# TLeconte/vdlm2dec

Measured on AMD Instinct MI355X. Metric: IQ MS/s demodulated (8 ch, 2 MS/s cs16) + CRC-pass frame parity vs ref, higher is better.
Workload: dtype f32

## Files before the change

vdlm2dec_amd/csrc/vdl2gpu_scan.h:

```cpp
#ifndef VDL2GPU_SCAN_H
#define VDL2GPU_SCAN_H

#ifndef K2A_THREADS
#define K2A_THREADS 256
#endif
#ifndef K2A_TS
#define K2A_TS 1024
#endif
#ifndef K2A_WPE
#define K2A_WPE 6
#endif
#define K2A_POFF 132
#define K2A_XOFF (K2A_POFF + 16)
#define K2A_XMAX (2 * K2A_TS + K2A_XOFF)
#define K2X_WL 40
#define K2X_NT 256
#define K2X_CV 64
#define VDL2_ITEM_CAP 196608
#define VDL2_ITEM_PRIV 131072
#define VDL2_MAXWG 512
#define VDL2_REG_CAP 4096
#ifndef VDL2_REG_PAD
#define VDL2_REG_PAD 40
#endif
#ifndef VDL2_REG_GAP
#define VDL2_REG_GAP 96
#endif
#define VDL2_SEG_CAP 4096
#define VDL2_VERIFIED 0x7f000000
#define VDL2_SEED_ERR 7.0f

struct K2aDef {
	int n;
	int r;
	int lo, hi;
};

#define K2A_ITEM_WORDS 5
struct K2aItem { float4 w[K2A_ITEM_WORDS]; };

#define K2A_WU1 (K2A_TS + K2A_XOFF + 4)
#define K2A_XS_LEN (K2A_WU1 + K2A_TS + K2A_POFF + 4)
struct alignas(16) K2aShared {
	float2 xs[K2A_XS_LEN];
	float smf[72];
	unsigned it_used, it_limit;
	unsigned short pend[K2A_THREADS / 64][K2A_TS / (K2A_THREADS / 64)];
	unsigned long long prof[K2A_ST_SLOTS];
};
static_assert(K2A_WU1 % 2 == 0 && K2A_XS_LEN >= K2A_XMAX + 8 && (K2A_XMAX / 2 + 4) % 2 == 0, "16-byte reads of xs[] and wu[]");
static_assert(K2A_TS + K2A_POFF / 2 + 2 <= K2A_XS_LEN && K2A_WU1 >= K2A_TS + K2A_XOFF, "phasor areas");
static_assert(K2A_TS <= 1024, "pend[] holds an instant within the tile in ten bits");
#define K2A_XODD (K2A_XMAX / 2 + 4)

#define VDL2_SCREEN_R2 56.25f
#define VDL2_SCREEN_R22 42.25f
#define VDL2_SCREEN_R32 30.25f
#define VDL2_FIT_MARGIN 0.25f
#define VDL2_NB_MARGIN 0.1f
__device__ __forceinline__ float k2_fast_angle(float y, float x)
{
	const float ax = __builtin_fabsf(x), ay = __builtin_fabsf(y);
	const float mn = __builtin_fminf(ax, ay), mx = __builtin_fmaxf(ax, ay);
	const float t = mn * __builtin_amdgcn_rcpf(mx);
	const float s = t * t;
	float p = __fmaf_rn(s, -0.0117212f, 0.05265332f);
	p = __fmaf_rn(s, p, -0.11643287f);
	p = __fmaf_rn(s, p, 0.19354346f);
	p = __fmaf_rn(s, p, -0.33262347f);
	p = __fmaf_rn(s, p, 0.99997726f) * t;
	p = ay > ax ? 1.57079637f - p : p;
	p = x < 0.0f ? 3.14159274f - p : p;
	return __builtin_copysignf(p, y);
}

__device__ __forceinline__ v2f k2_rot(v2f acc, v2f u, float cx, float cy)
{
	acc = __builtin_elementwise_fma((v2f){cx, cx}, u, acc);
	return __builtin_elementwise_fma((v2f){-cy, cy}, u.yx, acc);
}


template <class PR> __device__ __forceinline__ void k2a_emit(PR p, int sc, long long dec_base, long long n, int r, int mode,
						  long long chk_lo, long long chk_hi, int *fail, int skip_r, int skip_par,
						  float p2err, float perr, float err, float pfr, unsigned *cntp, unsigned *ovf, Cand *cl)
{
	if (mode >= SURV_PROBE && perr < VDL2_SEED_ERR && err > perr) {
		const unsigned kk = atomicAdd(p.ctl + CTL_NSEED0(p) + sc, 1u);
		if (kk < VDL2_CAND_CAP)
			p.seeds[(size_t)sc * VDL2_CAND_CAP + kk] = (int)(n - dec_base);
	}
	if (mode == SURV_SEEDS_NEVER_SET)
		return;
	if (!(perr < 4.0f && err > perr))
		return;
	if (mode == SURV_CANDS || mode == SURV_PROBE) {
		if (r == skip_r && (int)(n & 1) == skip_par)
			return;
		if (p.round == 0 && !p.full_scan && p2err < 4.0f && perr > p2err)
			return;
	} else {
		if (n < chk_lo || n >= chk_hi)
			return;
		atomicMin(fail, (int)(n - dec_base));
		const unsigned kc = atomicAdd(cntp, 1u);
		if (kc < VDL2_CAND_CAP) {
			Cand cd;
			cd.nrel = (int)(n - dec_base);
			cd.r = r;
			cd.p2err = p2err;
			cd.perr = perr;
			cd.err = err;
			cd.pfr = pfr;
			cl[kc] = cd;
			p.clhead[(size_t)sc * VDL2_CAND_CAP + kc] = cl_pack(0, CL_INVALID, 0, 0, 0, 0, 0);
		} else
			*ovf = 1u;
		return;
	}
	const unsigned kk = atomicAdd(cntp, 1u);
	if (kk < VDL2_CAND_CAP) {
		Cand cd;
		cd.nrel = (int)(n - dec_base);
		cd.r = r;
		cd.p2err = p2err;
		cd.perr = perr;
		cd.err = err;
		cd.pfr = pfr;
		cl[kk] = cd;
	} else
		*ovf = 1u;
}

__device__ __forceinline__ void k2a_tables(K2aShared &sh)
{
	for (int i = threadIdx.x; i < 72; i += K2A_THREADS)
		sh.smf[i] = (i < 65) ? d_tab(c_mflt, i) : 0.0f;
	if (threadIdx.x == 0) {
		sh.it_used = 0;
		sh.it_limit = 0xffffffffu;
	}
	__syncthreads();
}


__device__ __forceinline__ void k2a_append(K2aShared &sh, const K2Params &p, int sc, bool pass, int n_rel, int r, int lo, int hi, const float2 (&uu)[16], bool odd, int mode, int *fail)
{
	const unsigned long long m = __ballot(pass);
	if (m == 0)
		return;
	const unsigned lane_rank = __builtin_amdgcn_mbcnt_hi((unsigned)(m >> 32), __builtin_amdgcn_mbcnt_lo((unsigned)m, 0u));
	const unsigned cnt = (unsigned)__popcll(m);
	unsigned base = 0, stride = 0;
	if (lane_rank == 0 && pass) {
		const unsigned pch = (unsigned)p.surv_pch;
		const unsigned off = atomicAdd(&sh.it_used, cnt);
		if (off + cnt <= pch) {
			base = blockIdx.x * pch * K2A_ITEM_WORDS + off;
			stride = pch;
		} else {
			atomicMin(&sh.it_limit, off);
			const unsigned priv = (unsigned)p.surv_nwg * pch;
			const unsigned off2 = atomicAdd(p.ctl + CTL_NSURV0(p) + p.surv_slot * p.nstreams * VDL2_CS + sc, cnt);
			stride = p.item_cap - priv;
			const unsigned room = (p.surv_common_cap > 0 && (unsigned)p.surv_common_cap < stride) ? (unsigned)p.surv_common_cap : stride;
			base = (off2 + cnt <= room) ? priv * K2A_ITEM_WORDS + off2 : 0xffffffffu;
			if (base == 0xffffffffu)
				atomicMax(p.ctl + CTL_NSURVLIM0(p) + p.surv_slot * p.nstreams * VDL2_CS + sc, ~off2);
		}
	}
	const int lead = __builtin_ctzll(m);
	base = (unsigned)__builtin_amdgcn_readlane((int)base, lead);
	stride = (unsigned)__builtin_amdgcn_readlane((int)stride, lead);
	if (!pass)
		return;
	if (base != 0xffffffffu) {
		float4 *dst = reinterpret_cast<float4 *>(p.items) + (size_t)sc * p.item_cap * K2A_ITEM_WORDS + base + lane_rank;
		dst[0] = make_float4(__int_as_float(n_rel), __int_as_float(r | (odd ? 0x100 : 0)), __int_as_float(lo), __int_as_float(hi));
#pragma unroll
		for (int w = 0; w < 4; ++w) {
			typedef short s2 __attribute__((ext_vector_type(2)));
			union { s2 v; int i; } c[4];
#pragma unroll
			for (int l = 0; l < 4; ++l)
				c[l].v = __builtin_amdgcn_cvt_pknorm_i16(uu[4 * w + l].x, uu[4 * w + l].y);
			dst[(size_t)(1 + w) * stride] = make_float4(__int_as_float(c[0].i), __int_as_float(c[1].i), __int_as_float(c[2].i), __int_as_float(c[3].i));
		}
	} else if (mode == SURV_VERIFY)
		atomicMin(fail, 0);
	else
// ... 294 lines not shown
		v2f xe[10], xo[10];
#pragma unroll
		for (int i = 0; i < 5; ++i) {
			xe[2 * i] = e[i].xy;
			xe[2 * i + 1] = e[i].zw;
			xo[2 * i] = o[i].xy;
			xo[2 * i + 1] = o[i].zw;
		}
#pragma unroll
		for (int m = 0; m < 9; ++m) {
			acc0 = __builtin_elementwise_fma(xe[m], (v2f){mf[2 * m], mf[2 * m]}, acc0);
			acc1 = __builtin_elementwise_fma(xe[m + 1], (v2f){mf[2 * m], mf[2 * m]}, acc1);
			if (m < 8) {
				acc0 = __builtin_elementwise_fma(xo[m], (v2f){mf[2 * m + 1], mf[2 * m + 1]}, acc0);
				acc1 = __builtin_elementwise_fma(xo[m + 1], (v2f){mf[2 * m + 1], mf[2 * m + 1]}, acc1);
			}
		}
	} else {
		const v4f *pe = reinterpret_cast<const v4f *>(&sh.xs[q0]);
		v4f e[9];
#pragma unroll
		for (int i = 0; i < 9; ++i)
			e[i] = pe[i];
		v2f x[18];
#pragma unroll
		for (int i = 0; i < 9; ++i) {
			x[2 * i] = e[i].xy;
			x[2 * i + 1] = e[i].zw;
		}
#pragma unroll
		for (int j = 0; j < 17; ++j) {
			acc0 = __builtin_elementwise_fma(x[j], (v2f){mf[j], mf[j]}, acc0);
			acc1 = __builtin_elementwise_fma(x[j + 1], (v2f){mf[j], mf[j]}, acc1);
		}
	}
}

__device__ __forceinline__ v2f k2a_unit(v2f a)
{
	const float n2 = __fmaf_rn(a.x, a.x, a.y * a.y);
	v2f w = a * __frsqrt_rn(n2);
	if (!(n2 >= 1e-30f && n2 <= 1e30f)) {
		const float bad = (a.x == 0.0f && a.y == 0.0f) ? 0.0f : __builtin_nanf("");
		w = (v2f){1.0f + bad, bad};
	}
	return w;
}

__device__ __forceinline__ float k2a_lane_from(int byte_addr, float v)
{
	return __int_as_float(__builtin_amdgcn_ds_bpermute(byte_addr, __float_as_int(v)));
}

template <int S> __device__ void k2a_tile(K2aShared &sh, const K2Params &p, int sc, long long dec_base, long long nbase,
					   int cnt, unsigned rmask, int mode, long long chk_lo, long long chk_hi, int *fail,
					   int skip_r = -1, int skip_par = 0)
{
	const int tid = threadIdx.x;
	constexpr int PH = K2A_POFF / S;
	constexpr int LSTR = 8 / S;
	constexpr int E2 = 2 / S, E4 = 4 / S;
	constexpr int KH = LSTR / 2;
	constexpr int PPW = 64 - KH;
	constexpr int PPI = (K2A_THREADS / 64) * PPW;
	constexpr int NIT = ((K2A_TS + PH + 1) / 2 + PPI - 1) / PPI;
	constexpr int NL = (S * (K2A_TS - 1) + 1 + K2A_XOFF + K2A_THREADS - 1) / K2A_THREADS;
	static_assert(K2A_POFF == S * PH, "phase history must be a whole number of instants");
	float2 *const wu = (S != 1) ? sh.xs : sh.xs + K2A_WU1;
	const int nx = S * (cnt - 1) + 1 + K2A_XOFF;
	const bool prof = p.dbg && (mode == SURV_PROBE || (mode == SURV_CANDS && S == 1 && !p.full_scan && !p.full_round)) && tid == 0 && (blockIdx.x & 7) == 0;
	long long tq = prof ? clock64() : 0;
#define K2A_STAMP(slot) do { if (prof) { const long long tn = clock64(); sh.prof[slot] += (unsigned long long)(tn - tq); tq = tn; } } while (0)
	const int pbase = (S == 2) ? (tid & 1) * K2A_XODD + (tid >> 1) : tid;
	constexpr int pstep = K2A_THREADS / S;
	{
		const float2 *x = p.dec + (size_t)sc * p.cap + (nbase - K2A_XOFF - dec_base);
		float2 v[NL];
#pragma unroll
		for (int k = 0; k < NL; ++k)
			if (tid + k * K2A_THREADS < nx)
				v[k] = x[tid + k * K2A_THREADS];
		K2A_STAMP(K2A_ST_TILES_OR_WAIT);
#pragma unroll
		for (int k = 0; k < NL; ++k)
			if (tid + k * K2A_THREADS < nx)
				sh.xs[pbase + k * pstep] = v[k];
	}
	K2A_STAMP(K2A_ST_PARK);
	__syncthreads();
	K2A_STAMP(K2A_ST_STAGE_IN);
	const int npairs = (cnt + PH + 1) / 2;
	const int wv = tid >> 6, ln = tid & 63;
	const int src_lane = (ln - KH) * 4;
#pragma unroll 1
	for (int r = 0; r < 4; ++r) {
		if (!(rmask & (1u << r)))
			continue;
		float mf[17];
#pragma unroll
		for (int j = 0; j < 17; ++j)
			mf[j] = __int_as_float(__builtin_amdgcn_readfirstlane(__float_as_int(sh.smf[r + 4 * j])));
		float4 hold[NIT];
#pragma unroll
		for (int it = 0; it < NIT; ++it) {
			const int pw = it * PPI + wv * PPW;
			if (pw >= npairs) {
				hold[it] = make_float4(0.0f, 0.0f, 0.0f, 0.0f);
				continue;
			}
			int q0 = 2 * (pw + ln - KH);
			q0 = q0 < 0 ? 0 : (q0 > K2A_TS + PH - 2 ? K2A_TS + PH - 2 : q0);
			v2f acc[2];
			k2a_fir2<S>(sh, q0, mf, acc[0], acc[1]);
			const v2f w0 = k2a_unit(acc[0]), w1 = k2a_unit(acc[1]);
			const float p0x = k2a_lane_from(src_lane, w0.x), p0y = k2a_lane_from(src_lane, w0.y);
			const float p1x = k2a_lane_from(src_lane, w1.x), p1y = k2a_lane_from(src_lane, w1.y);
			hold[it] = make_float4(__fmaf_rn(w0.x, p0x, w0.y * p0y), __fmaf_rn(w0.y, p0x, -(w0.x * p0y)),
					       __fmaf_rn(w1.x, p1x, w1.y * p1y), __fmaf_rn(w1.y, p1x, -(w1.x * p1y)));
			__builtin_amdgcn_sched_barrier(0);
		}
		K2A_STAMP(K2A_ST_FIR_UNIT);
		if (S != 1)
			__syncthreads();
		K2A_STAMP(K2A_ST_BARRIER_SAMPLES);
#pragma unroll
		for (int it = 0; it < NIT; ++it) {
			const int q0 = 2 * (it * PPI + wv * PPW + ln - KH);
			if (ln >= KH && q0 >= LSTR && q0 < cnt + PH)
				*reinterpret_cast<float4 *>(&wu[q0]) = hold[it];
		}
		K2A_STAMP(K2A_ST_STEPS);
		__syncthreads();
		unsigned npend = 0;
		for (int i0 = 0; i0 < cnt; i0 += K2A_THREADS) {
			const int i = i0 + tid;
			const int j = (i < cnt ? i : cnt - 1) + E2;
			const float2 *uq = &wu[PH - E4 + j - 15 * LSTR];
			float2 uu[16];
#pragma unroll
			for (int l = 0; l < 16; ++l)
				uu[l] = uq[l * LSTR];
			constexpr int kq[16] = {7, 4, 5, 3, 7, 6, 1, 3, 6, 0, 5, 2, 1, 2, 0, 4};
			v2f s4[4] = {{0.0f, 0.0f}, {0.0f, 0.0f}, {0.0f, 0.0f}, {0.0f, 0.0f}};
#pragma unroll
			for (int l = 0; l < 16; ++l) {
				const v2f u = {uu[l].x, uu[l].y};
				const int g = ((kq[l] & 1) << 1) | ((kq[l] >> 1) & 1);
				if (kq[l] & 4)
					s4[g] -= u;
				else
					s4[g] += u;
			}
			const v2f pa = {s4[0].x - s4[1].y, s4[0].y + s4[1].x};
			const v2f qa = {s4[2].x - s4[3].y, s4[2].y + s4[3].x};
			constexpr float RH = 0.70710678118654752f;
			const v2f acc = {__fmaf_rn(qa.x - qa.y, RH, pa.x), __fmaf_rn(qa.x + qa.y, RH, pa.y)};
			const float r2 = __fmaf_rn(acc.x, acc.x, acc.y * acc.y);
			bool pass = i < cnt && !(r2 <= VDL2_SCREEN_R2);
			if (mode == SURV_CANDS && r == skip_r && (int)((nbase + S * (j - E4)) & 1) == skip_par)
				pass = false;
			const unsigned long long m = __ballot(pass);
			if (m != 0) {
				if (pass)
					sh.pend[wv][npend + __builtin_amdgcn_mbcnt_hi((unsigned)(m >> 32), __builtin_amdgcn_mbcnt_lo((unsigned)m, 0u))] =
						(unsigned short)(i | (!(r2 == r2) ? 0x8000 : 0));
				npend += (unsigned)__popcll(m);
			}
		}
		for (unsigned b = 0; b < npend; b += 64) {
			const bool on = b + (unsigned)ln < npend;
			const int e = on ? (int)sh.pend[wv][b + (unsigned)ln] : 0;
			const int j = (e & 0x3ff) + E2;
			const float2 *uq = &wu[PH - E4 + j - 15 * LSTR];
			float2 uu[16];
#pragma unroll
			for (int l = 0; l < 16; ++l)
				uu[l] = uq[l * LSTR];
			const long long n_abs = nbase + S * (j - E4);
			k2a_append(sh, p, sc, on, (int)(n_abs - dec_base), r, (mode == SURV_VERIFY) ? (int)(chk_lo - dec_base) : 0,
				   (mode == SURV_VERIFY) ? (int)(chk_hi - dec_base) : 0, uu, (e & 0x8000) != 0, mode, fail);
		}
		K2A_STAMP(K2A_ST_SCREEN);
		K2A_STAMP(K2A_ST_SCREEN_END);
		__syncthreads();
		K2A_STAMP(K2A_ST_BARRIER_TILE);
		if (prof)
			sh.prof[K2A_ST_PASSES] += 1ull;
	}
#undef K2A_STAMP
}

__global__ __launch_bounds__(K2A_THREADS) __attribute__((amdgpu_waves_per_eu(K2A_WPE, 8)))
void k2a_probe(K2Params p)
{
	__shared__ K2aShared sh;
	const int c = blockIdx.y, s = (int)blockIdx.z;
	const int sc = s * VDL2_CS + c;
	const long long dec_base = p.dec_base;
	const long long avail_end = dec_base + VDL2_CARRY_FRAMES + p.J;
	if (p.force_serial)
		return;
	if (p.round > 0 && (!p.full_round || p.fail[sc] >= VDL2_VERIFIED))
		return;
	if (threadIdx.x < K2A_ST_SLOTS)
		sh.prof[threadIdx.x] = 0;
	k2a_tables(sh);
	if (p.full_scan || p.full_round) {
		const long long step = (long long)gridDim.x * K2A_TS;
		for (long long n0 = p.scan_lo + (long long)blockIdx.x * K2A_TS; n0 < avail_end; n0 += step) {
			const int nt = (int)((avail_end - n0 < K2A_TS) ? (avail_end - n0) : K2A_TS);
			k2a_tile<1>(sh, p, sc, dec_base, n0, nt, 0xfu, SURV_CANDS, 0, 0, nullptr);
		}
		k2a_tail(sh, sc);
		return;
	}
	const unsigned rmask = 1u << p.probe_r;
	const long long step = 2LL * gridDim.x * K2A_TS;
	for (long long n0 = p.scan_lo + 2LL * blockIdx.x * K2A_TS; n0 < avail_end; n0 += step) {
		const long long left = (avail_end - n0 + 1) / 2;
		const int nt = (int)(left < K2A_TS ? left : K2A_TS);
		k2a_tile<2>(sh, p, sc, dec_base, n0, nt, rmask, SURV_PROBE, 0, 0, nullptr);
	}
	k2a_tail(sh, sc);
	if (p.dbg && threadIdx.x < K2A_ST_SLOTS && sh.prof[threadIdx.x])
		atomicAdd(p.dbg + K2_DBG_PROBE_STAGE0 + threadIdx.x, sh.prof[threadIdx.x]);
}

#define WGS_NBK 2048
#define WGS_MAXB 48
struct WgSortShared {
	unsigned long long tmp[VDL2_CAND_CAP];
	unsigned start[WGS_NBK + 1], cur[WGS_NBK];
	unsigned part[64];
	unsigned maxb;
};

template <int NT> __device__ void wg_sort_u64(unsigned long long *keys, WgSortShared &ws, int n, int tshift, unsigned range)
{
	const int tid = threadIdx.x;
	int bsh = 0;
	while ((range >> bsh) >= WGS_NBK)
		++bsh;
	for (int b = tid; b < WGS_NBK; b += NT)
		ws.cur[b] = 0;
	if (tid == 0)
		ws.maxb = 0;
	__syncthreads();
	for (int i = tid; i < n; i += NT) {
		unsigned b = (unsigned)(keys[i] >> tshift) >> bsh;
		b = b < WGS_NBK ? b : WGS_NBK - 1;
		const unsigned k = atomicAdd(&ws.cur[b], 1u);
		if (k + 1 > WGS_MAXB)
			ws.maxb = 1;
	}
	__syncthreads();
	if (ws.maxb) {
		int npow = 1;
		while (npow < n)
			npow <<= 1;
		for (int i = n + tid; i < npow; i += NT)
			keys[i] = ~0ull;
		__syncthreads();
		for (int k = 2; k <= npow; k <<= 1)
			for (int j = k >> 1; j > 0; j >>= 1) {
				for (int i = tid; i < npow; i += NT) {
					const int l = i ^ j;
					if (l > i) {
						const unsigned long long a0 = keys[i], b0 = keys[l];
						if ((a0 > b0) == ((i & k) == 0)) {
							keys[i] = b0;
							keys[l] = a0;
						}
					}
				}
// ... 106 lines not shown
				continue;
			int j = i;
			while (j + 1 < ncand && key[j + 1] - key[j] <= VDL2_REG_GAP)
				++j;
			int lo = key[i] - VDL2_REG_PAD, hi = key[j] + VDL2_REG_PAD + 1;
			lo = lo < lo_lim ? lo_lim : lo;
			hi = hi > hi_lim ? hi_lim : hi;
			if (hi <= lo)
				continue;
			const int nchunk = (hi - lo + K2A_TS - 1) / K2A_TS;
			const int base = atomicAdd(&s_nreg, nchunk);
			for (int k = 0; k < nchunk; ++k)
				if (base + k < VDL2_REG_CAP) {
					const int q = lo + k * K2A_TS;
					regs[base + k] = make_int2(q, (hi - q < K2A_TS) ? hi - q : K2A_TS);
				}
		}
		__syncthreads();
#ifdef VDL2GPU_TESTHOOKS
		if (K2_REG_LIM(p) < VDL2_REG_CAP && s_nreg > K2_REG_LIM(p)) {
			const int n = s_nreg < VDL2_REG_CAP ? s_nreg : VDL2_REG_CAP, lim = K2_REG_LIM(p);
			for (int i = tid; i < n; i += K2R_NT)
				key64[i] = ((unsigned long long)(unsigned)regs[i].x << 32) | (unsigned)regs[i].y;
			__syncthreads();
			for (int i = tid; i < n; i += K2R_NT) {
				const int x = (int)(key64[i] >> 32);
				int rank = 0;
				for (int j = 0; j < n; ++j)
					rank += ((int)(key64[j] >> 32) < x) ? 1 : 0;
				const int k = (int)(((long long)rank * lim + n - 1) / n);
				if (k < lim && (int)((long long)k * n / lim) == rank)
					regs[k] = make_int2(x, (int)(key64[i] & 0xffffffffu));
			}
			__syncthreads();
		}
#endif
		if (tid == 0) {
			const int n = s_nreg;
			p.ctl[CTL_NREG0(p) + sc] = (unsigned)(n > K2_REG_LIM(p) ? K2_REG_LIM(p) : n);
			if (n > K2_REG_LIM(p))
				K2_COUNT(p, K2_DBG_ESC_REG);
			p.ctl[CTL_NSEED0(p) + sc] = 0;
		}
	}
}

#ifndef K2A_WPE_REGION
#define K2A_WPE_REGION 5
#endif
__global__ __launch_bounds__(K2A_THREADS) __attribute__((amdgpu_waves_per_eu(K2A_WPE_REGION, 8)))
void k2a_region(K2Params p)
{
	__shared__ K2aShared sh;
	const int c = blockIdx.y, s = (int)blockIdx.z;
	const int sc = s * VDL2_CS + c;
	if (p.force_serial || p.full_scan)
		return;
#ifdef VDL2GPU_TESTHOOKS
	if (p.test_noregion && p.round == 0)
		return;
#endif
	const unsigned nreg = p.ctl[CTL_NREG0(p) + sc];
	if (blockIdx.x >= nreg)
		return;
	const long long dec_base = p.dec_base;
	const int2 *regs = p.regs + (size_t)sc * VDL2_REG_CAP;
	const int skip_r = p.probe_r, skip_par = p.probe_par;
	if (threadIdx.x < K2A_ST_SLOTS)
		sh.prof[threadIdx.x] = 0;
	k2a_tables(sh);
	const bool prof = p.dbg && threadIdx.x == 0 && (blockIdx.x & 7) == 0;
	const long long t0 = prof ? clock64() : 0;
	for (unsigned k = blockIdx.x; k < nreg; k += gridDim.x) {
		const int2 rg = regs[k];
		k2a_tile<1>(sh, p, sc, dec_base, dec_base + rg.x, rg.y, 0xfu, SURV_CANDS, 0, 0, nullptr, skip_r, skip_par);
		if (prof)
			sh.prof[K2A_ST_INSTANTS] += (unsigned long long)rg.y;
	}
	const long long t1 = prof ? clock64() : 0;
	if (prof)
		sh.prof[K2A_ST_TILES_OR_WAIT] += (unsigned long long)(t1 - t0);
	k2a_tail(sh, sc);
	if (p.dbg && threadIdx.x < K2A_ST_SLOTS && sh.prof[threadIdx.x])
		atomicAdd(p.dbg + K2_DBG_REGION_STAGE0 + threadIdx.x, sh.prof[threadIdx.x]);
}

#ifndef K2A_VRUN
#define K2A_VRUN 4
#endif
#ifndef K2A_VGRID_RESIDENT
#define K2A_VGRID_RESIDENT 1
#endif
#define K2A_VITEMS 64

__device__ __forceinline__ int k2a_vseg(const Seg *segs, int k, int nseg, int p_lo, int t_end, int &lo, int &hi, int &r)
{
	lo = hi = r = 0;
	if (k >= nseg)
		return 0;
	const Seg g = segs[k];
	lo = g.lo > p_lo ? g.lo : p_lo;
	lo += (lo ^ g.lo) & 1;
	hi = g.hi < t_end ? g.hi : t_end;
	r = g.r & 3;
	if (g.hi <= g.lo || hi <= lo) {
		hi = lo;
		return 0;
	}
	return ((hi - lo + 1) / 2 + K2A_TS - 1) / K2A_TS;
}

__device__ __forceinline__ int k2a_vscan(int v, int *s_w, int &total)
{
	int incl = v;
	incl += __builtin_amdgcn_update_dpp(0, incl, 0x111, 0xf, 0xf, false);
	incl += __builtin_amdgcn_update_dpp(0, incl, 0x112, 0xf, 0xf, false);
	incl += __builtin_amdgcn_update_dpp(0, incl, 0x114, 0xf, 0xf, false);
	incl += __builtin_amdgcn_update_dpp(0, incl, 0x118, 0xf, 0xf, false);
	incl += __builtin_amdgcn_update_dpp(0, incl, 0x142, 0xa, 0xf, false);
	incl += __builtin_amdgcn_update_dpp(0, incl, 0x143, 0xc, 0xf, false);
	__syncthreads();
	if ((threadIdx.x & 63) == 63)
		s_w[threadIdx.x >> 6] = incl;
	__syncthreads();
	int base = 0, tot = 0;
#pragma unroll
	for (int w = 0; w < K2A_THREADS / 64; ++w) {
		const int t = s_w[w];
// ... 31 lines not shown
}

__global__ __launch_bounds__(K2A_THREADS) __attribute__((amdgpu_waves_per_eu(K2A_WPE, 8)))
void k2a_verify(K2Params p)
{
	__shared__ K2aShared sh;
	__shared__ int s_w[K2A_THREADS / 64];
	__shared__ int4 s_item[K2A_VITEMS];
	const int tid = threadIdx.x;
	const int c = blockIdx.y, s = (int)blockIdx.z;
	const int sc = s * VDL2_CS + c;
	if (p.force_serial || p.full_scan || p.full_round)
		return;
	if (p.round > 0 && !p.redo[sc])
		return;
	const long long dec_base = p.dec_base;
	const int t_end = (int)(VDL2_CARRY_FRAMES + p.J);
	int nseg = (int)p.ctl[CTL_NSEG0(p) + sc];
	if (tid == 0 && blockIdx.x == 0 && (nseg < 0 || nseg > K2_SEG_LIM(p)))
		K2_COUNT(p, K2_DBG_ESC_SEG);
	nseg = nseg < 0 || nseg > K2_SEG_LIM(p) ? K2_SEG_LIM(p) : nseg;
	const Seg *segs = p.segs + (size_t)sc * VDL2_SEG_CAP;
	if (nseg == 0)
		return;
	const int p_lo = (int)(p.cs[sc].pos - dec_base);
	int lo0, hi0, r0;
	const int n0 = k2a_vseg(segs, tid, nseg, p_lo, t_end, lo0, hi0, r0);
	int T;
	{
		int mine = n0;
		for (int k = K2A_THREADS + tid; k < nseg; k += K2A_THREADS) {
			int lo, hi, r;
			mine += k2a_vseg(segs, k, nseg, p_lo, t_end, lo, hi, r);
		}
		k2a_vscan(mine, s_w, T);
	}
	const int G = (int)gridDim.x;
	const int q = (T + G - 1) / G;
	int ch = (int)blockIdx.x;
	int a = ch * q;
	if (a >= T)
		return;
	int c_end = a + q < T ? a + q : T;
	k2a_tables(sh);
	int b = a + K2A_VITEMS < c_end ? a + K2A_VITEMS : c_end;
	k2a_vitems<true>(segs, nseg, p_lo, t_end, a, b, lo0, hi0, r0, n0, s_w, s_item);
	for (;;) {
		const int ni = b - a;
		if (p.dbg && tid < ni)
			atomicAdd(p.dbg + K2_DBG_VERIFY_INSTANTS, (unsigned long long)((s_item[tid].y - s_item[tid].x + 1) / 2));
		for (int i = 0; i < ni; ++i) {
			const int4 it = s_item[i];
			k2a_tile<2>(sh, p, sc, dec_base, dec_base + it.x, (it.y - it.x + 1) / 2, 1u << it.z, SURV_VERIFY, dec_base + it.x, dec_base + it.y,
				    p.fail + sc);
		}
		a = b;
		if (a >= c_end) {
			ch += G;
			a = ch * q;
			if (a >= T)
				break;
			c_end = a + q < T ? a + q : T;
		}
		b = a + K2A_VITEMS < c_end ? a + K2A_VITEMS : c_end;
		__syncthreads();
		k2a_vitems<false>(segs, nseg, p_lo, t_end, a, b, 0, 0, 0, 0, s_w, s_item);
	}
	k2a_tail(sh, sc);
}

#endif
```

vdlm2dec_amd/csrc/vdl2gpu_types.h:

```cpp
#ifndef VDL2GPU_TYPES_H
#define VDL2GPU_TYPES_H


#include <hip/hip_runtime.h>
#include <stdint.h>
#include "vdl2_math.h"
#include "../../include/vdl2gpu.h"

#define VDL2_CS 8
#ifndef VDL2_NSET
#define VDL2_NSET 3
#endif
#define VDL2_NRING VDL2_NSET
#define VDL2_NSLAB (VDL2_NSET + 1)
static_assert(VDL2_NSET >= 3 && VDL2_NSET <= 4, "three bits of a record handle name its slab");
#define VDL2_HIST 160
#define VDL2_NPH 68
#define VDL2_STEADY 68
#define VDL2_MAXSYM 5456
#define VDL2_SERIAL_BELOW 4096
#define VDL2_CARRY_FRAMES 49152
#define VDL2_LONGEST_BURST 43592
#define VDL2_LEV_GUARD 512
#define VDL2_LEV_NEVAL 256
// ... 205 lines not shown
	vdl2gpu_soft_t *soft;
	RingCount *outc;
	OutCounters::Totals *outc_total;
	unsigned *fmask;
	int full_round;
	int mini_round;
	int sel_reserved;
	unsigned rec_cap;
	int force_serial;
	int prim_drop;
	int full_scan;
	int test_noregion;
	int2 *regs;
	Seg *segs;
	int *fail;
	int *redo;
	int round;
	ChanState *cs_out;
	int *skey;
	unsigned short *sidx;
	unsigned short *prim;
	uint8_t *onchain;
	K2Slog *slog;
	int2 *win;
	int *seeds;
	struct K2aItem *items;
	unsigned item_cap;
	unsigned item_priv;
	int surv_pch, surv_nwg;
	int surv_common_cap;
	int surv_slot;
	int surv_mode;
	int surv_skip;
	int drain_slot;
	int drain_mode, drain_skip;
	int drain_pch, drain_nwg;
	unsigned long long *dbg;
	HeadTap *headtap;
	unsigned *headtap_n;
	unsigned headtap_cap;
	vdl2gpu_carrier_t *carrier;
#ifdef VDL2GPU_TESTHOOKS
	int lim_reg, lim_seg, lim_vis, lim_win, lim_merge, lim_slog;
#endif
};
enum K2Dbg {
	K2_DBG_K2B_RING_TICKS = 0, K2_DBG_K2B_REST_TICKS, K2_DBG_K2B_SAMPLED, K2_DBG_K2B_TRIG, K2_DBG_K2B_EVAL, K2_DBG_K2B_MAX_TICKS,
	K2_DBG_K2B_STEADY, K2_DBG_K2B_REJ, K2_DBG_K2B_ORD_TICKS0 = 8, K2_DBG_K2B_ORD_COUNT0 = 12,
	K2_DBG_K2C_LOAD_TICKS = 16, K2_DBG_K2C_TABLES_TICKS, K2_DBG_K2C_WALK_TICKS, K2_DBG_K2C_PUBLISH_TICKS, K2_DBG_K2C_CALLS,
	K2_DBG_REPAIRED = 24, K2_DBG_K2C_REPLAYS, K2_DBG_K2C_NONSTEADY, K2_DBG_K2C_CANDS, K2_DBG_K2C_VISITED, K2_DBG_K2C_SERIAL_SAMPLES,
	K2_DBG_VERIFY_INSTANTS = 30, K2_DBG_PROBE_STAGE0 = 32, K2_DBG_REGION_STAGE0 = 48,
	K2_DBG_ESC_REG = 64, K2_DBG_ESC_SEG, K2_DBG_ESC_VIS, K2_DBG_ESC_WIN, K2_DBG_ESC_MERGE, K2_DBG_ESC_SLOG, K2_DBG_ESC_STAGE,
	K2_DBG_INV_B_CLUSTER, K2_DBG_INV_B_DECODE, K2_DBG_INV_B_RECORD, K2_DBG_INV_A, K2_DBG_ESC_MERGE_SORT,
	K2_DBG_ESC_PATCH_ABANDON, K2_DBG_CHK_B_CLUSTER, K2_DBG_CHK_B_DECODE, K2_DBG_CHK_B_RECORD, K2_DBG_CHK_A
};
enum K2aStage {
	K2A_ST_STAGE_IN = 0, K2A_ST_FIR_UNIT, K2A_ST_BARRIER_SAMPLES, K2A_ST_STEPS, K2A_ST_SCREEN, K2A_ST_UNUSED5, K2A_ST_UNUSED6, K2A_ST_UNUSED7,
	K2A_ST_SCREEN_END, K2A_ST_BARRIER_TILE, K2A_ST_UNUSED10, K2A_ST_PASSES , K2A_ST_TILES_OR_WAIT, K2A_ST_PARK, K2A_ST_UNUSED14,
	K2A_ST_INSTANTS , K2A_ST_SLOTS
};
static_assert(K2A_ST_SLOTS == 16 && K2_DBG_REGION_STAGE0 == K2_DBG_PROBE_STAGE0 + K2A_ST_SLOTS && K2_DBG_ESC_REG == K2_DBG_REGION_STAGE0 + K2A_ST_SLOTS,
	      "the two scans' stage slots lie between the resolver's counters and the test build's");
#ifdef VDL2GPU_TESTHOOKS
#define K2_REG_LIM(p) ((p).lim_reg)
#define K2_SEG_LIM(p) ((p).lim_seg)
#define K2_VIS_LIM(p) ((p).lim_vis)
#define K2_WIN_LIM(p) ((p).lim_win)
#define K2_MERGE_LIM(p) ((p).lim_merge)
#define K2_SLOG_LIM(p) ((p).lim_slog)
#define VDL2_DBG_WORDS 96
#define K2_COUNT(p, slot) do { if ((p).dbg) atomicAdd((p).dbg + (slot), 1ull); } while (0)
#else
#define K2_REG_LIM(p) VDL2_REG_CAP
#define K2_SEG_LIM(p) VDL2_SEG_CAP
#define K2_VIS_LIM(p) K2C_VIS
#define K2_WIN_LIM(p) VDL2_WIN_CAP
#define K2_MERGE_LIM(p) K2S_MERGE
#define K2_SLOG_LIM(p) VDL2_SLOG_CAP
#define VDL2_DBG_WORDS 64
#define K2_COUNT(p, slot) do { } while (0)
#endif
#define CTL_OUT 0
#define CTL_OUT_OVF 1
#define CTL_STAGE 2
#define CTL_TICKET 3
#define CTL_STAGE_OVF 4
#define CTL_CAND0 8
enum { VDL2_SURV_PROBE = 0, VDL2_SURV_REGION = 1, VDL2_SURV_VERIFY = 2 , VDL2_SURV_FULL = 7, VDL2_SURV_SLOTS = 8 };
enum { CTL_B_CAND = 0, CTL_B_CANDOVF, CTL_B_NREG, CTL_B_NSEG, CTL_B_NSEL, CTL_B_NPRIM, CTL_B_NSEED, CTL_B_NCLUST,
       CTL_B_NSURV, CTL_B_SELBASE = CTL_B_NSURV + VDL2_SURV_SLOTS, CTL_B_NSEL1, CTL_B_SELBASE1,
       CTL_B_NSURVLIM, CTL_B_NWIN = CTL_B_NSURVLIM + VDL2_SURV_SLOTS, CTL_B_NSLOG, CTL_B_END };
#define CTL_BLOCK(p, b) (CTL_CAND0 + (b) * (p).nstreams * VDL2_CS)
#define CTL_CANDOVF0(p) CTL_BLOCK(p, CTL_B_CANDOVF)
#define CTL_NREG0(p) CTL_BLOCK(p, CTL_B_NREG)
#define CTL_NSEG0(p) CTL_BLOCK(p, CTL_B_NSEG)
#define CTL_NSEL0(p) CTL_BLOCK(p, CTL_B_NSEL)
#define CTL_NPRIM0(p) CTL_BLOCK(p, CTL_B_NPRIM)
#define CTL_NSEED0(p) CTL_BLOCK(p, CTL_B_NSEED)
#define CTL_NCLUST0(p) CTL_BLOCK(p, CTL_B_NCLUST)
#define CTL_NSURV0(p) CTL_BLOCK(p, CTL_B_NSURV)
#define CTL_SELBASE0(p) CTL_BLOCK(p, CTL_B_SELBASE)
#define CTL_NSEL1(p) CTL_BLOCK(p, CTL_B_NSEL1)
#define CTL_SELBASE1(p) CTL_BLOCK(p, CTL_B_SELBASE1)
#define CTL_NSURVLIM0(p) CTL_BLOCK(p, CTL_B_NSURVLIM)
#define CTL_NWIN0(p) CTL_BLOCK(p, CTL_B_NWIN)
#define CTL_NSLOG0(p) CTL_BLOCK(p, CTL_B_NSLOG)
#define VDL2_CTL_WORDS(nsc) (CTL_CAND0 + CTL_B_END * (size_t)(nsc))
// ... 47 lines not shown
```

vdlm2dec_amd/lib.py:

```python
from __future__ import annotations

import ctypes as C
import os

_HERE = os.path.dirname(os.path.abspath(__file__))
LIB_PATH = os.path.join(_HERE, "libvdl2gpu.so")
LIB_TEST_PATH = os.path.join(_HERE, "libvdl2gpu_test.so")

FMT = {"cu8": 0, "cs16": 1, "cf32": 2, "f32": 3, "cs8": 4, "s16": 5}
SAMPLE_BYTES = {"cu8": 2, "cs16": 4, "cf32": 8, "f32": 4, "cs8": 2, "s16": 2}
MEM_HOST, MEM_DEVICE = 0, 1
F_KEEP_DEC = 1
F_SERIAL = 2
F_FULLSCAN = 4
F_TEST_NOREGION = 8
F_FRAMES = 16
F_RTL_QUIRK = 32
F_DEBUG_HEADS = 64
F_LEVELS = 128
F_SOFT_RS = 256
F_EXACT_FO = 512
F_CARRIER = 1024
F_BLOCK_REPORT = 2048
ROW_NONE, ROW_CLEAN, ROW_REF, ROW_SOFT2, ROW_SOFT4, ROW_FAIL = range(6)
ROW_FEEDBACK = 6
F_FEEDBACK = 4096
F_ALL_FRAMES = 8192
BLK_ALL_FRAMES = 1
F_RAW_FLAGS = 16384
BLK_RAW_FLAGS = 4
F_SYMCLK = 32768
SYMCLK_SEG, SYMCLK_SEGS = 256, 22
CL_STEADY, CL_DEFER_FIRST, CL_NONSTEADY = 0, 1, 2


DBG = {
    "K2B_RING_TICKS": 0, "K2B_REST_TICKS": 1, "K2B_SAMPLED": 2, "K2B_TRIG": 3, "K2B_EVAL": 4, "K2B_MAX_TICKS": 5,
    "K2B_STEADY": 6, "K2B_REJ": 7, "K2B_ORD_TICKS0": 8, "K2B_ORD_COUNT0": 12,
    "K2C_LOAD_TICKS": 16, "K2C_TABLES_TICKS": 17, "K2C_WALK_TICKS": 18, "K2C_PUBLISH_TICKS": 19, "K2C_CALLS": 20,
    "REPAIRED": 24, "K2C_REPLAYS": 25, "K2C_NONSTEADY": 26, "K2C_CANDS": 27, "K2C_VISITED": 28, "K2C_SERIAL_SAMPLES": 29,
    "VERIFY_INSTANTS": 30, "PROBE_STAGE0": 32, "REGION_STAGE0": 48,
    "ESC_REG": 64, "ESC_SEG": 65, "ESC_VIS": 66, "ESC_WIN": 67, "ESC_MERGE": 68, "ESC_SLOG": 69, "ESC_STAGE": 70,
    "INV_B_CLUSTER": 71, "INV_B_DECODE": 72, "INV_B_RECORD": 73, "INV_A": 74, "ESC_MERGE_SORT": 75,
    "ESC_PATCH_ABANDON": 76, "CHK_B_CLUSTER": 77, "CHK_B_DECODE": 78, "CHK_B_RECORD": 79, "CHK_A": 80,
}
DBG_STAGES = ("stage_in", "fir_unit", "barrier_samples", "steps", "screen", "unused5", "unused6", "unused7",
              "screen_end", "barrier_tile", "unused10", "passes", "tiles_or_wait", "park", "unused14", "instants")
DBG_WORDS, DBG_WORDS_TEST = 64, 96


def dbg_stages(counters, base):
    return ", ".join("%s %d" % (name, counters[base + i]) for i, name in enumerate(DBG_STAGES) if counters[base + i])


def cl_unpack(packed):
    p = int(packed) & 0xffffffff
    return p & 3, p >> 2 & 3, p >> 4 & 15, p >> 8 & 255, p >> 16 & 255, p >> 24 & 255


EXPORTS = (
    "vdl2gpu_abi_version", "vdl2gpu_create", "vdl2gpu_destroy", "vdl2gpu_push", "vdl2gpu_sync",
    "vdl2gpu_ring_init", "vdl2gpu_ring_acquire", "vdl2gpu_ring_commit",
    "vdl2gpu_poll", "vdl2gpu_poll_ready", "vdl2gpu_poll_levels", "vdl2gpu_poll_levels_ready", "vdl2gpu_poll_soft", "vdl2gpu_poll_soft_ready", "vdl2gpu_poll_carrier", "vdl2gpu_poll_carrier_ready", "vdl2gpu_poll_report", "vdl2gpu_poll_report_ready", "vdl2gpu_poll_feedback", "vdl2gpu_poll_feedback_ready", "vdl2gpu_poll_symclk", "vdl2gpu_poll_symclk_ready", "vdl2gpu_pending", "vdl2gpu_inflight", "vdl2gpu_get_stats", "vdl2gpu_get_timing", "vdl2gpu_get_host_profile", "vdl2gpu_last_error",
    "vdl2gpu_strerror", "vdl2gpu_burst_to_msgblk", "vdl2gpu_decode_blocks", "vdl2gpu_decode_blocks_soft", "vdl2gpu_decode_blocks_report", "vdl2gpu_decode_blocks_feedback", "vdl2gpu_decode_blocks_ex", "vdl2gpu_poll_frames", "vdl2gpu_poll_frames_ready", "reversebits", "vdl2gpu_lo_len", "vdl2gpu_lo_table", "vdl2gpu_plan",
    "vdl2gpu_exact_fo_tables", "vdl2gpu_exact_fo_index", "vdl2gpu_carrier_from_sums", "vdl2gpu_symclk_from_sums",
    "vdl2gpu_choose_fc_rtl", "vdl2gpu_choose_fc_air",
    "vdl2gpu_debug_dec", "vdl2gpu_debug_k1", "vdl2gpu_debug_lo", "vdl2gpu_debug_atan2f", "vdl2gpu_debug_rs", "vdl2gpu_debug_counters", "vdl2gpu_debug_cands", "vdl2gpu_debug_clheads", "vdl2gpu_debug_fail", "vdl2gpu_debug_segs", "vdl2gpu_debug_heads",
)


class ChanT(C.Structure):
    _fields_ = [("chn", C.c_int32), ("Fr", C.c_int32), ("Fo", C.c_int32)]


class ConfigT(C.Structure):
    _fields_ = [("struct_size", C.c_uint32), ("sdrinrate", C.c_uint32), ("sdrclk", C.c_uint32),
                ("fmt", C.c_int32), ("nbch", C.c_int32), ("nstreams", C.c_int32),
                ("chan", C.POINTER(ChanT)), ("max_push", C.c_uint64), ("device", C.c_int32),
                ("max_bursts", C.c_uint32), ("flags", C.c_uint32)]


class BurstT(C.Structure):
    _fields_ = [("stream", C.c_int32), ("chn", C.c_int32), ("Fr", C.c_int32), ("nbrow", C.c_int32),
                ("nlbyte", C.c_int32), ("df", C.c_float), ("ppm", C.c_float),
                ("trig_dec", C.c_int64), ("end_dec", C.c_int64), ("trig_sample", C.c_int64),
                ("end_sample", C.c_int64), ("data", (C.c_uint8 * 255) * 8)]


class LevelT(C.Structure):
    _fields_ = [("sig_dbfs", C.c_float), ("noise_dbfs", C.c_float), ("sig_power", C.c_float), ("noise_power", C.c_float),
                ("sym_first_dec", C.c_int64), ("nsym", C.c_int32), ("subphase", C.c_int32), ("noise_blocks", C.c_int32),
                ("reserved", C.c_int32)]


class SoftT(C.Structure):
    _fields_ = [("rel", (C.c_uint8 * 255) * 8), ("reserved", C.c_uint8 * 8)]

# ... 192 lines not shown
```

Measured before the change: 181,100.

## Compute sync-word screen correlation with half-precision MFMA matrix products

Replaces the per-thread 16-tap complex correlation screen in the scan tile with fp16 MFMA 16x16x32 products. Phasors are written to half-precision planes in LDS, and a small shared table holds the sync-symbol coefficients. Each wavefront screens 256 instants with four matrix ops and compacts the pending list through ballots. To absorb fp16 error the screen threshold is lowered slightly, and a test-build check counts instants the f32 screen would flag but the new path misses. The change adds LDS usage (an extra shared array for S=1) and a precision risk near the threshold.

```diff
diff --git a/vdlm2dec_amd/csrc/vdl2gpu_scan.h b/vdlm2dec_amd/csrc/vdl2gpu_scan.h
--- a/vdlm2dec_amd/csrc/vdl2gpu_scan.h
+++ b/vdlm2dec_amd/csrc/vdl2gpu_scan.h
@@ -41,19 +41,32 @@
 
 #define K2A_WU1 (K2A_TS + K2A_XOFF + 4)
 #define K2A_XS_LEN (K2A_WU1 + K2A_TS + K2A_POFF + 4)
+#define K2A_SCB 21
 struct alignas(16) K2aShared {
 	float2 xs[K2A_XS_LEN];
 	float smf[72];
 	unsigned it_used, it_limit;
 	unsigned short pend[K2A_THREADS / 64][K2A_TS / (K2A_THREADS / 64)];
 	unsigned long long prof[K2A_ST_SLOTS];
+	float4 scb[2 * K2A_SCB];
 };
+template <int S> struct K2aHalf {
+	static constexpr int LSTR = 8 / S;
+	static constexpr int HOFF = 4 * LSTR - (K2A_POFF / S - 2 / S - 15 * LSTR);
+	static constexpr int USED = K2A_TS / LSTR + 4 + 16;
+	static constexpr int PLEN = (S == 2) ? 324 : 148;
+	static_assert(HOFF >= 0 && PLEN >= USED && PLEN % 4 == 0, "planes");
+};
+struct alignas(16) K2aHalf1 { unsigned hu[K2aHalf<1>::LSTR * K2aHalf<1>::PLEN]; };
+static_assert(K2aHalf<2>::LSTR * K2aHalf<2>::PLEN * 4 <= (K2A_XS_LEN - K2A_WU1) * 8, "S = 2: the half-precision phasors fit behind wu[]");
 static_assert(K2A_WU1 % 2 == 0 && K2A_XS_LEN >= K2A_XMAX + 8 && (K2A_XMAX / 2 + 4) % 2 == 0, "16-byte reads of xs[] and wu[]");
 static_assert(K2A_TS + K2A_POFF / 2 + 2 <= K2A_XS_LEN && K2A_WU1 >= K2A_TS + K2A_XOFF, "phasor areas");
 static_assert(K2A_TS <= 1024, "pend[] holds an instant within the tile in ten bits");
 #define K2A_XODD (K2A_XMAX / 2 + 4)
 
-#define VDL2_SCREEN_R2 56.25f
+#define VDL2_SCREEN_DELTA 0.01f
+#define VDL2_SCREEN_R2 ((7.5f - VDL2_SCREEN_DELTA) * (7.5f - VDL2_SCREEN_DELTA))
+#define VDL2_SCREEN_R2_F32 56.25f
 #define VDL2_SCREEN_R22 42.25f
 #define VDL2_SCREEN_R32 30.25f
 #define VDL2_FIT_MARGIN 0.25f
@@ -132,10 +145,45 @@
 		*ovf = 1u;
 }
 
+constexpr int K2A_KQ[16] = {7, 4, 5, 3, 7, 6, 1, 3, 6, 0, 5, 2, 1, 2, 0, 4};
+constexpr unsigned long long k2a_kq_packed()
+{
+	unsigned long long v = 0;
+	for (int l = 0; l < 16; ++l)
+		v |= (unsigned long long)K2A_KQ[l] << (4 * l);
+	return v;
+}
+constexpr unsigned long long K2A_KQ_PACKED = k2a_kq_packed();
+
+typedef _Float16 v2h __attribute__((ext_vector_type(2)));
+typedef _Float16 v8h __attribute__((ext_vector_type(8)));
+typedef float v4f32 __attribute__((ext_vector_type(4)));
+__device__ __forceinline__ unsigned k2a_half2(float re, float im)
+{
+	union { v2h v; unsigned u; } c;
+	c.v = (v2h){(_Float16)re, (_Float16)im};
+	return c.u;
+}
+__device__ __forceinline__ float k2a_cos8(int k)
+{
+	const float m = (k & 1) ? 0.70710678118654752f : ((k & 2) ? 0.0f : 1.0f);
+	return (((k + 5) & 7) < 3) ? -m : m;
+}
+
 __device__ __forceinline__ void k2a_tables(K2aShared &sh)
 {
 	for (int i = threadIdx.x; i < 72; i += K2A_THREADS)
 		sh.smf[i] = (i < 65) ? d_tab(c_mflt, i) : 0.0f;
+	for (int i = threadIdx.x; i < 2 * K2A_SCB * 4; i += K2A_THREADS) {
+		const int t = i / (K2A_SCB * 4), d = (i % (K2A_SCB * 4)) / 4 - 4 + (i & 3);
+		float cr = 0.0f, ci = 0.0f;
+		if (d >= 0 && d < 16) {
+			const int k = (int)(K2A_KQ_PACKED >> (4 * d)) & 7;
+			cr = k2a_cos8(k);
+			ci = k2a_cos8((k + 6) & 7);
+		}
+		reinterpret_cast<unsigned *>(sh.scb)[i] = t ? k2a_half2(ci, cr) : k2a_half2(cr, -ci);
+	}
 	if (threadIdx.x == 0) {
 		sh.it_used = 0;
 		sh.it_limit = 0xffffffffu;
@@ -536,9 +584,43 @@
 	return __int_as_float(__builtin_amdgcn_ds_bpermute(byte_addr, __float_as_int(v)));
 }
 
+#ifdef VDL2GPU_TESTHOOKS
+__device__ __forceinline__ void k2a_screen_check(const K2Params &p, bool valid, bool passed, const float2 *uq, int lstr)
+{
+	if (!p.dbg)
+		return;
+	bool miss = false;
+	if (valid) {
+		v2f s4[4] = {{0.0f, 0.0f}, {0.0f, 0.0f}, {0.0f, 0.0f}, {0.0f, 0.0f}};
+#pragma unroll
+		for (int l = 0; l < 16; ++l) {
+			const v2f u = {uq[l * lstr].x, uq[l * lstr].y};
+			const int kq = (int)(K2A_KQ_PACKED >> (4 * l)) & 7;
+			const int g = ((kq & 1) << 1) | ((kq >> 1) & 1);
+			if (kq & 4)
+				s4[g] -= u;
+			else
+				s4[g] += u;
+		}
+		const v2f pa = {s4[0].x - s4[1].y, s4[0].y + s4[1].x};
+		const v2f qa = {s4[2].x - s4[3].y, s4[2].y + s4[3].x};
+		constexpr float RH = 0.70710678118654752f;
+		const v2f acc = {__fmaf_rn(qa.x - qa.y, RH, pa.x), __fmaf_rn(qa.x + qa.y, RH, pa.y)};
+		const float r2 = __fmaf_rn(acc.x, acc.x, acc.y * acc.y);
+		miss = r2 > VDL2_SCREEN_R2_F32 && !passed;
+	}
+	const unsigned long long mv = __ballot(valid), mm = __ballot(miss);
+	if ((threadIdx.x & 63) == 0) {
+		atomicAdd(p.dbg + K2_DBG_CHK_SCREEN, (unsigned long long)__popcll(mv));
+		if (mm)
+			atomicAdd(p.dbg + K2_DBG_INV_SCREEN, (unsigned long long)__popcll(mm));
+	}
+}
+#endif
+
 template <int S> __device__ void k2a_tile(K2aShared &sh, const K2Params &p, int sc, long long dec_base, long long nbase,
 					   int cnt, unsigned rmask, int mode, long long chk_lo, long long chk_hi, int *fail,
-					   int skip_r = -1, int skip_par = 0)
+					   K2aHalf1 *half1, int skip_r = -1, int skip_par = 0)
 {
 	const int tid = threadIdx.x;
 	constexpr int PH = K2A_POFF / S;
@@ -551,6 +633,9 @@
 	constexpr int NL = (S * (K2A_TS - 1) + 1 + K2A_XOFF + K2A_THREADS - 1) / K2A_THREADS;
 	static_assert(K2A_POFF == S * PH, "phase history must be a whole number of instants");
 	float2 *const wu = (S != 1) ? sh.xs : sh.xs + K2A_WU1;
+	typedef K2aHalf<S> H;
+	unsigned *const hu = (S != 1) ? reinterpret_cast<unsigned *>(sh.xs + K2A_WU1) : half1->hu;
+	static_assert((K2A_THREADS / 64) * 256 == K2A_TS && 16 % LSTR == 0, "a wavefront's four matrix products are 256 consecutive instants of the tile");
 	const int nx = S * (cnt - 1) + 1 + K2A_XOFF;
 	const bool prof = p.dbg && (mode == SURV_PROBE || (mode == SURV_CANDS && S == 1 && !p.full_scan && !p.full_round)) && tid == 0 && (blockIdx.x & 7) == 0;
 	long long tq = prof ? clock64() : 0;
@@ -607,48 +692,76 @@
 		if (S != 1)
 			__syncthreads();
 		K2A_STAMP(K2A_ST_BARRIER_SAMPLES);
+		int tdh = tid;
+		asm volatile("" : "+v"(tdh));
 #pragma unroll
 		for (int it = 0; it < NIT; ++it) {
 			const int q0 = 2 * (it * PPI + wv * PPW + ln - KH);
 			if (ln >= KH && q0 >= LSTR && q0 < cnt + PH)
 				*reinterpret_cast<float4 *>(&wu[q0]) = hold[it];
+			const int qh = 2 * (it * PPI + (tdh >> 6) * PPW + (tdh & 63) - KH);
+			if ((tdh & 63) >= KH && qh >= LSTR) {
+				const int h0 = qh + H::HOFF, h1 = h0 + 1;
+				if (h0 < LSTR * H::USED)
+					hu[(h0 % LSTR) * H::PLEN + h0 / LSTR] = (qh < cnt + PH) ? k2a_half2(hold[it].x, hold[it].y) : 0u;
+				if (h1 < LSTR * H::USED)
+					hu[(h1 % LSTR) * H::PLEN + h1 / LSTR] = (qh + 1 < cnt + PH) ? k2a_half2(hold[it].z, hold[it].w) : 0u;
+			}
 		}
 		K2A_STAMP(K2A_ST_STEPS);
 		__syncthreads();
 		unsigned npend = 0;
-		for (int i0 = 0; i0 < cnt; i0 += K2A_THREADS) {
-			const int i = i0 + tid;
-			const int j = (i < cnt ? i : cnt - 1) + E2;
-			const float2 *uq = &wu[PH - E4 + j - 15 * LSTR];
-			float2 uu[16];
-#pragma unroll
-			for (int l = 0; l < 16; ++l)
-				uu[l] = uq[l * LSTR];
-			constexpr int kq[16] = {7, 4, 5, 3, 7, 6, 1, 3, 6, 0, 5, 2, 1, 2, 0, 4};
-			v2f s4[4] = {{0.0f, 0.0f}, {0.0f, 0.0f}, {0.0f, 0.0f}, {0.0f, 0.0f}};
-#pragma unroll
-			for (int l = 0; l < 16; ++l) {
-				const v2f u = {uu[l].x, uu[l].y};
-				const int g = ((kq[l] & 1) << 1) | ((kq[l] >> 1) & 1);
-				if (kq[l] & 4)
-					s4[g] -= u;
-				else
-					s4[g] += u;
+		const int ibase = wv * 256;
+		if (ibase < cnt) {
+			int tds = tid;
+			asm volatile("" : "+v"(tds));
+			const int G = (tds >> 4) & 3, o = tds & 15;
+			const unsigned *ap = hu + (o % LSTR) * H::PLEN + (ibase / LSTR + 16 * (o / LSTR) + 4) + 4 * G;
+			const v8h a0 = *reinterpret_cast<const v8h *>(ap), a1 = *reinterpret_cast<const v8h *>(ap + 16);
+			const int d0 = 4 * G - o;
+			const v8h *bt = reinterpret_cast<const v8h *>(sh.scb) + (d0 + 4 < 0 ? 0 : d0 + 4);
+			const v8h *bu = reinterpret_cast<const v8h *>(sh.scb) + (d0 + 20 > K2A_SCB - 1 ? K2A_SCB - 1 : d0 + 20);
+			v4f32 yr = {0.0f, 0.0f, 0.0f, 0.0f}, yi = {0.0f, 0.0f, 0.0f, 0.0f};
+			yr = __builtin_amdgcn_mfma_f32_16x16x32_f16(a0, bt[0], yr, 0, 0, 0);
+			yi = __builtin_amdgcn_mfma_f32_16x16x32_f16(a0, bt[K2A_SCB], yi, 0, 0, 0);
+			yr = __builtin_amdgcn_mfma_f32_16x16x32_f16(a1, bu[0], yr, 0, 0, 0);
+			yi = __builtin_amdgcn_mfma_f32_16x16x32_f16(a1, bu[K2A_SCB], yi, 0, 0, 0);
+			const int il = ibase + ((S == 2) ? 64 * G + 4 * o : 128 * (G >> 1) + 8 * o + 4 * (G & 1));
+			bool ps[4], od[4];
+			unsigned long long m[4];
+#pragma unroll
+			for (int k = 0; k < 4; ++k) {
+				const int i = il + k;
+				const float r2 = __fmaf_rn(yr[k], yr[k], yi[k] * yi[k]);
+				ps[k] = i < cnt && !(r2 <= VDL2_SCREEN_R2);
+				od[k] = !(r2 == r2);
+#ifdef VDL2GPU_TESTHOOKS
+				k2a_screen_check(p, i < cnt, ps[k], &wu[PH - E2 + i - 15 * LSTR], LSTR);
+#endif
+				if (mode == SURV_CANDS && r == skip_r && (int)((nbase + S * (i - E2)) & 1) == skip_par)
+					ps[k] = false;
+				m[k] = __ballot(ps[k]);
 			}
-			const v2f pa = {s4[0].x - s4[1].y, s4[0].y + s4[1].x};
-			const v2f qa = {s4[2].x - s4[3].y, s4[2].y + s4[3].x};
-			constexpr float RH = 0.70710678118654752f;
-			const v2f acc = {__fmaf_rn(qa.x - qa.y, RH, pa.x), __fmaf_rn(qa.x + qa.y, RH, pa.y)};
-			const float r2 = __fmaf_rn(acc.x, acc.x, acc.y * acc.y);
-			bool pass = i < cnt && !(r2 <= VDL2_SCREEN_R2);
-			if (mode == SURV_CANDS && r == skip_r && (int)((nbase + S * (j - E4)) & 1) == skip_par)
-				pass = false;
-			const unsigned long long m = __ballot(pass);
-			if (m != 0) {
-				if (pass)
-					sh.pend[wv][npend + __builtin_amdgcn_mbcnt_hi((unsigned)(m >> 32), __builtin_amdgcn_mbcnt_lo((unsigned)m, 0u))] =
-						(unsigned short)(i | (!(r2 == r2) ? 0x8000 : 0));
-				npend += (unsigned)__popcll(m);
+			if ((m[0] | m[1] | m[2] | m[3]) != 0) {
+				unsigned lo, hi;
+				if (S == 2) {
+					lo = (tds & 32) ? 0xffffffffu : (1u << (tds & 31)) - 1u;
+					hi = (tds & 32) ? (1u << (tds & 31)) - 1u : 0u;
+				} else {
+					const unsigned in32 = ((1u << o) - 1u) * 0x10001u | ((G & 1) ? 1u << o : 0u);
+					lo = (G >> 1) ? 0xffffffffu : in32;
+					hi = (G >> 1) ? in32 : 0u;
+				}
+				unsigned at = 0;
+#pragma unroll
+				for (int k = 0; k < 4; ++k) {
+					at += (unsigned)__popc((unsigned)m[k] & lo) + (unsigned)__popc((unsigned)(m[k] >> 32) & hi);
+					npend += (unsigned)__popcll(m[k]);
+				}
+#pragma unroll
+				for (int k = 0; k < 4; ++k)
+					if (ps[k])
+						sh.pend[wv][at++] = (unsigned short)((il + k) | (od[k] ? 0x8000 : 0));
 			}
 		}
 		for (unsigned b = 0; b < npend; b += 64) {
@@ -678,6 +791,7 @@
 void k2a_probe(K2Params p)
 {
 	__shared__ K2aShared sh;
+	__shared__ K2aHalf1 half1;
 	const int c = blockIdx.y, s = (int)blockIdx.z;
 	const int sc = s * VDL2_CS + c;
 	const long long dec_base = p.dec_base;
@@ -693,7 +807,7 @@
 		const long long step = (long long)gridDim.x * K2A_TS;
 		for (long long n0 = p.scan_lo + (long long)blockIdx.x * K2A_TS; n0 < avail_end; n0 += step) {
 			const int nt = (int)((avail_end - n0 < K2A_TS) ? (avail_end - n0) : K2A_TS);
-			k2a_tile<1>(sh, p, sc, dec_base, n0, nt, 0xfu, SURV_CANDS, 0, 0, nullptr);
+			k2a_tile<1>(sh, p, sc, dec_base, n0, nt, 0xfu, SURV_CANDS, 0, 0, nullptr, &half1);
 		}
 		k2a_tail(sh, sc);
 		return;
@@ -703,7 +817,7 @@
 	for (long long n0 = p.scan_lo + 2LL * blockIdx.x * K2A_TS; n0 < avail_end; n0 += step) {
 		const long long left = (avail_end - n0 + 1) / 2;
 		const int nt = (int)(left < K2A_TS ? left : K2A_TS);
-		k2a_tile<2>(sh, p, sc, dec_base, n0, nt, rmask, SURV_PROBE, 0, 0, nullptr);
+		k2a_tile<2>(sh, p, sc, dec_base, n0, nt, rmask, SURV_PROBE, 0, 0, nullptr, nullptr);
 	}
 	k2a_tail(sh, sc);
 	if (p.dbg && threadIdx.x < K2A_ST_SLOTS && sh.prof[threadIdx.x])
@@ -916,6 +1030,7 @@
 void k2a_region(K2Params p)
 {
 	__shared__ K2aShared sh;
+	__shared__ K2aHalf1 half1;
 	const int c = blockIdx.y, s = (int)blockIdx.z;
 	const int sc = s * VDL2_CS + c;
 	if (p.force_serial || p.full_scan)
@@ -937,7 +1052,7 @@
 	const long long t0 = prof ? clock64() : 0;
 	for (unsigned k = blockIdx.x; k < nreg; k += gridDim.x) {
 		const int2 rg = regs[k];
-		k2a_tile<1>(sh, p, sc, dec_base, dec_base + rg.x, rg.y, 0xfu, SURV_CANDS, 0, 0, nullptr, skip_r, skip_par);
+		k2a_tile<1>(sh, p, sc, dec_base, dec_base + rg.x, rg.y, 0xfu, SURV_CANDS, 0, 0, nullptr, &half1, skip_r, skip_par);
 		if (prof)
 			sh.prof[K2A_ST_INSTANTS] += (unsigned long long)rg.y;
 	}
@@ -1075,7 +1190,7 @@
 		for (int i = 0; i < ni; ++i) {
 			const int4 it = s_item[i];
 			k2a_tile<2>(sh, p, sc, dec_base, dec_base + it.x, (it.y - it.x + 1) / 2, 1u << it.z, SURV_VERIFY, dec_base + it.x, dec_base + it.y,
-				    p.fail + sc);
+				    p.fail + sc, nullptr);
 		}
 		a = b;
 		if (a >= c_end) {
diff --git a/vdlm2dec_amd/csrc/vdl2gpu_types.h b/vdlm2dec_amd/csrc/vdl2gpu_types.h
--- a/vdlm2dec_amd/csrc/vdl2gpu_types.h
+++ b/vdlm2dec_amd/csrc/vdl2gpu_types.h
@@ -281,7 +281,8 @@
 	K2_DBG_VERIFY_INSTANTS = 30, K2_DBG_PROBE_STAGE0 = 32, K2_DBG_REGION_STAGE0 = 48,
 	K2_DBG_ESC_REG = 64, K2_DBG_ESC_SEG, K2_DBG_ESC_VIS, K2_DBG_ESC_WIN, K2_DBG_ESC_MERGE, K2_DBG_ESC_SLOG, K2_DBG_ESC_STAGE,
 	K2_DBG_INV_B_CLUSTER, K2_DBG_INV_B_DECODE, K2_DBG_INV_B_RECORD, K2_DBG_INV_A, K2_DBG_ESC_MERGE_SORT,
-	K2_DBG_ESC_PATCH_ABANDON, K2_DBG_CHK_B_CLUSTER, K2_DBG_CHK_B_DECODE, K2_DBG_CHK_B_RECORD, K2_DBG_CHK_A
+	K2_DBG_ESC_PATCH_ABANDON, K2_DBG_CHK_B_CLUSTER, K2_DBG_CHK_B_DECODE, K2_DBG_CHK_B_RECORD, K2_DBG_CHK_A,
+	K2_DBG_CHK_SCREEN, K2_DBG_INV_SCREEN
 };
 enum K2aStage {
 	K2A_ST_STAGE_IN = 0, K2A_ST_FIR_UNIT, K2A_ST_BARRIER_SAMPLES, K2A_ST_STEPS, K2A_ST_SCREEN, K2A_ST_UNUSED5, K2A_ST_UNUSED6, K2A_ST_UNUSED7,
diff --git a/vdlm2dec_amd/lib.py b/vdlm2dec_amd/lib.py
--- a/vdlm2dec_amd/lib.py
+++ b/vdlm2dec_amd/lib.py
@@ -43,6 +43,7 @@
     "ESC_REG": 64, "ESC_SEG": 65, "ESC_VIS": 66, "ESC_WIN": 67, "ESC_MERGE": 68, "ESC_SLOG": 69, "ESC_STAGE": 70,
     "INV_B_CLUSTER": 71, "INV_B_DECODE": 72, "INV_B_RECORD": 73, "INV_A": 74, "ESC_MERGE_SORT": 75,
     "ESC_PATCH_ABANDON": 76, "CHK_B_CLUSTER": 77, "CHK_B_DECODE": 78, "CHK_B_RECORD": 79, "CHK_A": 80,
+    "CHK_SCREEN": 81, "INV_SCREEN": 82,
 }
 DBG_STAGES = ("stage_in", "fir_unit", "barrier_samples", "steps", "screen", "unused5", "unused6", "unused7",
               "screen_end", "barrier_tile", "unused10", "passes", "tiles_or_wait", "park", "unused14", "instants")
```

New measurement: 178,100. 0.984x the previous value.
